# timosachsenberg/specpride

Measured on AMD Instinct MI355X. Metric: clusters/sec (whole node) for medoid + binned consensus, higher is better.
Workload: dtype f64; 1 GPU; configs[4]: full pipeline (bin-mean consensus + medoid representative) on a PRIDE-scale clustered dataset of ~10M spectra, U{2..50} spectra/cluster, ~200 peaks/spectrum; clusters=385000, clusters_this_rank=385000, spectra_this_rank=10008913, parallelism=cluster-sharded x1, launcher=single process, gather=none (1 GPU: results stay in HBM)

## Files before the change

### specpride_amd/csrc/bin_mean.hip

```cpp
#pragma once
#include <utility>

#include "spx_device.hpp"

namespace spx {

struct BinMeanParams {
  double minimum, maximum, binsize, inv_binsize;
  int32_t apply_quorum;
  int32_t n_words;
};

template <class PrefixT, class CountT = uint32_t>
struct BinMeanState {
  unsigned long long* bitmap;
  PrefixT* wprefix;
  CountT* cnt;
  float* acc_i;
  float* acc_m;
  uint32_t* owner;
  int32_t* soff;
  double* prec;
  int* votes;
  int32_t* xch;
// ... 432 lines not shown
    w[4 * k] = q.x; w[4 * k + 1] = q.y; w[4 * k + 2] = q.z; w[4 * k + 3] = q.w;
  }
  static_assert(BR_MDW32 == 4 * BM_BLOCK, "one b128 of medoid words per thread");
  const uint4 mq = reinterpret_cast<const uint4*>(L.u.b.mdbits)[threadIdx.x];
  const uint32_t mw[4] = {mq.x, mq.y, mq.z, mq.w};
  int local = 0, mlocal = 0;
#pragma unroll
  for (int k = 0; k < BR_WPT; ++k) local += __popc(w[k]);
#pragma unroll
  for (int k = 0; k < 4; ++k) mlocal += __popc(mw[k]);
  int total;
  const int packed = block_exclusive_scan<BM_BLOCK, int, true, false>(local | (mlocal << 16), L.tmp, total);
  int base = packed & 0xFFFF, mbase = (int)((uint32_t)packed >> 16);
  uint2* dst = reinterpret_cast<uint2*>(L.u.b.pre) + threadIdx.x * (BR_WPT / 4);
#pragma unroll
  for (int k = 0; k < BR_WPT / 4; ++k) {
    uint32_t p[4];
#pragma unroll
    for (int i = 0; i < 4; ++i) { p[i] = (uint32_t)base; base += __popc(w[4 * k + i]); }
    dst[k] = make_uint2(p[0] | (p[1] << 16), p[2] | (p[3] << 16));
  }
  uint32_t mp[4];
#pragma unroll
  for (int i = 0; i < 4; ++i) { mp[i] = (uint32_t)mbase; mbase += __popc(mw[i]); }
  reinterpret_cast<uint2*>(L.u.b.mdpre)[threadIdx.x] = make_uint2(mp[0] | (mp[1] << 16), mp[2] | (mp[3] << 16));
  lds_barrier();
  *md_total = (int)((uint32_t)total >> 16);
  return total & 0xFFFF;
}

struct MdSide {
  double tol, inv_tol;
  int out, K;
  int32_t rlo, rhi;
};

template <class F>
__device__ __forceinline__ void reg_steps(int n, F&& f) {
  unrolled_while(n, f, std::make_integer_sequence<int, BR_NMAX>{});
}

template <bool kMd>
__device__ __forceinline__ int32_t bin_mean_reg_path_t(const CsrView& v, const BinMeanParams& P, BinRegSmem& L,
                                                       int64_t c, const PeaksOut& out, double* prec_out,
                                                       int32_t* charge_out, int32_t (&code)[BR_NMAX], MdSide* md) {
  const int tid = threadIdx.x, lane = lane_id(), wid = wave_id();
  constexpr int KM = kMd ? SPX_BR_KM_MD : BR_KM;
  constexpr int PFA = kMd ? SPX_BR_PFA_MD : BR_PFA;
  const int64_t s0 = v.cluster_off[c], s1 = v.cluster_off[c + 1], n64 = s1 - s0;
  if (n64 < 1 || n64 > BR_NMAX || P.n_words > BM_WMAX) return kNotHere;
  const int n = (int)n64;
  const int64_t p0 = v.spec_off[s0], p1 = v.spec_off[s1];
  if (p1 == p0 || p1 - p0 >= (int64_t(1) << 28)) return kNotHere;
  const int jl = lane < n ? lane : n - 1;
  const int32_t rlo = (int32_t)(v.spec_off[s0 + jl] - p0), rhi = (int32_t)(v.spec_off[s0 + jl + 1] - p0);
  const int32_t z0 = v.charge[s0];
  const bool mine = lane < n;
  const int32_t zl = v.charge[s0 + jl];
  const double pl = v.prec_mz[s0 + jl];
  if (__ballot(mine & ((rhi - rlo) > BM_FASTLEN)) != 0ull) return kNotHere;
  if (__ballot(mine & (zl != z0)) != 0ull) {
    if (tid == 0) { out.count[c] = 0; prec_out[c] = __longlong_as_double(0x7ff8000000000000ll); charge_out[c] = 0; }
    return kMixedCharge;
  }
  if (wid == 0 && mine) L.prec[lane] = pl;
  if constexpr (kMd) {
    md->rlo = rlo;
    md->rhi = rhi;
    reinterpret_cast<uint4*>(L.u.b.mdbits)[tid] = make_uint4(0u, 0u, 0u, 0u);
  }
  {
    uint4* z = reinterpret_cast<uint4*>(L.u.b.bits) + tid * (BR_WPT / 4);
#pragma unroll
    for (int k = 0; k < BR_WPT / 4; ++k) z[k] = make_uint4(0u, 0u, 0u, 0u);
    if (tid < kWave) {
      L.u.b.bits[BR_W32 + tid] = 0u;
      L.u.b.pre[BR_W32 + tid] = (uint16_t)(BM_DCAP + tid);
    }
  }
  lds_barrier();
  SPX_STAMP2(1, -1);

  const int fpos = wid * (kWave - 1) + lane;
  const bool owner = lane < kWave - 1;
  const __amdgpu_buffer_rsrc_t rmz = bf_rsrc(v.mz + p0, (int)(p1 - p0));
  const __amdgpu_buffer_rsrc_t rit = bf_rsrc(v.inten + p0, (int)(p1 - p0));
  auto boffb = [&](int j) -> int {
    const int jj = j < n ? j : n - 1;
    return (__builtin_amdgcn_readlane(rlo, jj) + fpos) * 8;
  };

  double mk[KM > 0 ? KM : 1];
  uint32_t* bm32 = L.u.b.bits;
  int bad = 0, mdout = 0;
  {
    double ra[PFA];
    int rl[PFA];
    auto fetch = [&](int j, double& m, int& len) __attribute__((always_inline)) {
      const int jj = j < n ? j : n - 1;
      const int a = __builtin_amdgcn_readlane(rlo, jj), e = __builtin_amdgcn_readlane(rhi, jj);
      const int k = a + fpos;
      len = e - a;
      m = bf_load(rmz, k * 8, 0);
// ... 107 lines not shown
  lds_barrier();
  for (int d = tid; d < D; d += BM_BLOCK) L.u.acc[d] = BinAcc{0.0f, 0.0f, 0u, 0u};
  lds_barrier();
  SPX_STAMP2(3, 2);

  reg_steps(n, [&](auto jc) __attribute__((always_inline)) {
    constexpr int j = decltype(jc)::value;
    double m;
    const double it = ri[j % BR_PFC];
    if constexpr (j < KM) m = mk[j];
    else m = rm[j % BR_PFC];
    const int bo = boffb(j + BR_PFC);
    if constexpr (j + BR_PFC >= KM) rm[j % BR_PFC] = bf_load(rmz, bo, 0);
    ri[j % BR_PFC] = bf_load(rit, bo, 0);
    const int slot = kMd ? code[j] & 0xFFFF : code[j];
    if constexpr (kMd && (j & 1)) {
      code[j - 1] = (int32_t)(((uint32_t)code[j - 1] >> 16) | ((uint32_t)code[j] & 0xFFFF0000u));
    }
    BinAcc a = L.u.acc[slot];
    a.i = (float)((double)a.i + it);
    a.m = (float)((double)a.m + m);
    a.n += 1u;
    L.u.acc[slot] = a;
    lds_barrier();
  });
  SPX_STAMP2(4, 3);

  const uint32_t quorum = P.apply_quorum ? (uint32_t)((double)n * 0.25) + 1u : 1u;
  const int total = emit_striped_f([&](int d) { return L.u.acc[d].n; }, [&](int d) { return L.u.acc[d].i; },
                                   [&](int d) { return L.u.acc[d].m; }, L.wcnt, D, quorum, out.mz + p0,
                                   out.inten + p0);
  if (tid == 0) {
    out.count[c] = total;
    charge_out[c] = z0;
    prec_out[c] = pw_sum_small([&](int64_t j) { return L.prec[j]; }, n) / (double)n;
  }
  return kOk;
}

using BinHeadSmem = BinRegSmem;
__device__ __forceinline__ int32_t bin_mean_head_path(const CsrView& v, const BinMeanParams& P, BinHeadSmem& L,
                                                      int64_t c, const PeaksOut& out, double* prec_out,
                                                      int32_t* charge_out) {
  int32_t code[BR_NMAX];
  return bin_mean_reg_path_t<false>(v, P, L, c, out, prec_out, charge_out, code, nullptr);
}

__global__ __launch_bounds__(BM_BLOCK, SPX_BR_MINW) void bin_mean_reg_kernel(CsrView v, BinMeanParams P, PeaksOut out,
                                                                             double* prec_out, int32_t* charge_out,
                                                                             int32_t* status, StripedList rest) {
  __shared__ BinHeadSmem L;
  const int64_t c = blockIdx.x;
  SPX_STAMP(0);
  const int32_t st = bin_mean_head_path(v, P, L, c, out, prec_out, charge_out);
  SPX_STAMP(6);
  if (threadIdx.x == 0) {
    if (st != kNotHere) status[c] = st;
    if (st == kNotHere || st == kDeferred) striped_push(rest, (int32_t)c);
  }
}

__global__ __launch_bounds__(BM_BLOCK, SPX_BM_MINW) void bin_mean_lds_kernel(CsrView v, BinMeanParams P, PeaksOut out,
                                                                double* prec_out, int32_t* charge_out,
                                                                int32_t* status, const int32_t* list,
                                                                const int32_t* n_list, int32_t* deferred,
                                                                int32_t* n_deferred) {
  __shared__ BinMeanSmem L;
// ... 78 lines not shown
```

### specpride_amd/csrc/fused.hip

```cpp
#include "bin_mean.hip"
#include "medoid.hip"

namespace spx {

#ifndef SPX_FU_MINW
#define SPX_FU_MINW 5
#endif

union FusedSmem {
  BinHeadSmem b;
  MedoidRegSmem<MD_BLOCK, MR_UMAX, MD_KWMAX> m;
};
static_assert(BM_BLOCK == MD_BLOCK, "one workgroup shape for both bodies");

template <class Defer>
__device__ __forceinline__ void medoid_from_codes(const CsrView& v, int64_t* rep, double* totals_out,
                                                  MedoidRegSmem<MD_BLOCK, MR_UMAX, MD_KWMAX>& L, int64_t c,
                                                  const int32_t (&code)[BR_NMAX], const MdSide& md,
                                                  const Defer& defer) {
  const int tid = threadIdx.x, lane = lane_id(), wid = wave_id();
  const int64_t s0 = v.cluster_off[c];
  const int n = (int)(v.cluster_off[c + 1] - s0);
  if (n <= 1) {
    if (tid == 0) {
      rep[c] = n == 1 ? s0 : -1;
      if (totals_out && n == 1) totals_out[s0] = 0.0;
    }
    return;
  }
  const int KW = ((md.K + 63) / 64) | 1;
  if (KW > MD_KWMAX) {
    if (tid == 0) defer(c, s0, n);
    return;
  }
  if (tid <= n) L.soff[tid] = tid < n ? md.rlo : md.rhi;
  for (int w = tid; w < n * KW; w += MD_BLOCK) L.u.a.rows[w] = 0ull;
  __syncthreads();
  const uint32_t swz_nw = 2u * (uint32_t)KW;
  const uint32_t swz_m = swz_nw >= 32u ? 31u : (1u << (31 - __clz((int)swz_nw))) - 1u;
  const int fpos = wid * (kWave - 1) + lane;
  const bool owner = lane < kWave - 1;
  reg_steps(n, [&](auto jc) __attribute__((always_inline)) {
    constexpr int j = decltype(jc)::value;
    const int len = __builtin_amdgcn_readlane(md.rhi, j) - __builtin_amdgcn_readlane(md.rlo, j);
    if (owner & (fpos < len)) {
      uint32_t col;
      if constexpr (j & 1) col = (uint32_t)code[j - 1] >> 16;
      else col = j + 1 < n ? (uint32_t)code[j] & 0xFFFFu : (uint32_t)code[j] >> 16;
      uint32_t wq = (col >> 5) + (col & swz_m);
      wq = min(wq, wq - swz_nw);
      atomicOr(reinterpret_cast<uint32_t*>(&L.u.a.rows[__mul24(j, KW)]) + wq, 1u << (col & 31));
    }
  });
  SPX_STAMP2(-1, 5);
  medoid_tail<MD_BLOCK, MR_UMAX, MD_KWMAX>(L, n, KW, s0, c, rep, totals_out);
}

__global__ __launch_bounds__(BM_BLOCK, SPX_FU_MINW) void bin_mean_medoid_kernel(
    CsrView v, BinMeanParams PB, PeaksOut out, double* prec_out, int32_t* charge_out, int32_t* status,
    StripedList bm_rest, MedoidParams PM, int64_t* rep, double* totals_out, StripedList md_wide) {
  __shared__ FusedSmem L;
  const int64_t c = blockIdx.x;
  SPX_STAMP2(-1, 0);
  int32_t code[BR_NMAX];
  MdSide md{PM.tol, PM.inv_tol, 1, 0, 0, 0};
  const int32_t st = bin_mean_reg_path_t<true>(v, PB, L.b, c, out, prec_out, charge_out, code, &md);
  if (threadIdx.x == 0) {
    if (st != kNotHere) status[c] = st;
    if (st == kNotHere || st == kDeferred) striped_push(bm_rest, (int32_t)c);
  }
  SPX_STAMP2(-1, 4);
  __syncthreads();
  auto defer = [&](int64_t cc, int64_t, int) {
    rep[cc] = -4;
    striped_push(md_wide, (int32_t)cc);
  };
  if (st == kOk && !md.out) {
    medoid_from_codes(v, rep, totals_out, L.m, c, code, md, defer);
  } else {
    medoid_small_body<MD_BLOCK, MR_UMAX, MD_KWMAX>(v, PM, rep, totals_out, L.m, c, defer);
  }
}

__global__ __launch_bounds__(kWave) void handoff_count_kernel(const int32_t* bm_counts, const int32_t* md_counts,
                                                              int32_t* out) {
  const int l = threadIdx.x;
  const int32_t a = wave_sum(bm_counts[l * kListLine]);
  const int32_t b = wave_sum(md_counts[l * kListLine]);
  if (l == 0) {
    out[0] = a;
    out[1] = b;
  }
}

}
```

### specpride_amd/csrc/medoid.hip

```cpp
#pragma once
#include <type_traits>

#include "spx_device.hpp"

namespace spx {

struct MedoidParams {
  double tol, inv_tol;
};

constexpr int MD_BLOCK = 256;
constexpr int MD_NMAX = 64;
#ifndef SPX_MD_KWMAX
#define SPX_MD_KWMAX 27
#endif
#ifndef SPX_MD_MINW
#define SPX_MD_MINW 7
#endif
#ifndef SPX_MD_MFMA_NMIN
#define SPX_MD_MFMA_NMIN 32
#endif
constexpr int MD_KWMAX = SPX_MD_KWMAX;


// ... 101 lines not shown
constexpr int MR_UMAX = 48;
constexpr int MR_PMAX = MR_UMAX * MD_BLOCK;
constexpr int MR_WMAX = 512;
constexpr int MR_TRI = MD_NMAX * (MD_NMAX + 1) / 2;

constexpr int MW_BLOCK = 512;
constexpr int MW_UMAX = 64;
constexpr int MW_PMAX = MW_UMAX * MW_BLOCK;
constexpr int MW_KWMAX = 95;

template <int BLOCK, int UMAX, int KWMAX>
struct MedoidRegSmem {
  union {
    struct {
      unsigned long long bits[MR_WMAX];
      uint32_t pre[MR_WMAX];
      unsigned long long rows[MD_NMAX * KWMAX];
      unsigned long long sbits[UMAX * BLOCK / 64];
      uint8_t spre[UMAX * BLOCK / 64];
    } a;
    double d[MR_TRI];
    struct {
      double d[MR_TRI];
      double col[MD_NMAX];
    } t;
  } u;
  int32_t soff[MD_NMAX + 1];
  double totals[MD_NMAX];
  int tmp[BLOCK / kWave + 1];
  long long red[4];
  int votes[2 * (BLOCK / kWave)];
};

template <int BLOCK, int UMAX, int KWMAX>
__device__ __forceinline__ void medoid_tail(MedoidRegSmem<BLOCK, UMAX, KWMAX>& L, int n, int KW, int64_t s0,
                                            int64_t c, int64_t* rep, double* totals_out) {
  constexpr int PMAX = UMAX * BLOCK;
  const int tid = threadIdx.x, lane = lane_id(), wid = wave_id();
  static_assert(PMAX <= 65536, "md_dist_r's exact range");
  if (tid < n) {
    const int p = L.soff[tid + 1] - L.soff[tid];
    L.totals[tid] = p > 0 ? 1.0 / (double)p : 0.0;
  }
  __syncthreads();
  SPX_STAMP2(4, -1);

  auto row_start = [&](int i) { return i * n - (i * (i - 1)) / 2; };
  bool mfma_p4 = false;
  if constexpr (BLOCK == MD_BLOCK) mfma_p4 = n > SPX_MD_MFMA_NMIN;
  if (mfma_p4) {
  {
    const int fr = lane & 31, fh = lane >> 5;
    const int ntile = n > 32 ? 3 : 1;
    const bool work = wid < ntile;
    const int ta = wid == 2 ? 1 : 0, tb = wid == 0 ? 0 : 1;
    md_f32x16 acc;
#pragma unroll
    for (int q = 0; q < 16; ++q) acc[q] = 0.0f;
    if (work) {
      const int ra = ta * 32 + fr, rb = tb * 32 + fr;
      const unsigned long long* pa = L.u.a.rows + (ra < n ? ra : 0) * KW;
      const unsigned long long* pb = L.u.a.rows + (rb < n ? rb : 0) * KW;
      const unsigned long long ma = ra < n ? ~0ull : 0ull, mb = rb < n ? ~0ull : 0ull;
      unsigned long long wa = pa[0] & ma, wb = pb[0] & mb;
      for (int w = 0; w < KW; ++w) {
        const int wn = w + 1 < KW ? w + 1 : w;
        const unsigned long long na = pa[wn] & ma, nb = pb[wn] & mb;
        acc = __builtin_amdgcn_mfma_scale_f32_32x32x64_f8f6f4(md_frag4(wa, fh), md_frag4(wb, fh), acc, 4, 4, 0, 0,
                                                              0, 0);
        wa = na;
        wb = nb;
      }
    }
    __syncthreads();
    if (work) {
      const int j = tb * 32 + fr;
#pragma unroll
      for (int q = 0; q < 16; ++q) {
// ... 10 lines not shown
    constexpr int PPT = (MD_NMAX * (MD_NMAX + 1) / 2 + BLOCK - 1) / BLOCK;
    const int NP = n * (n + 1) / 2;
    uint32_t pc[PPT];
    int pij[PPT];
#pragma unroll
    for (int q = 0; q < PPT; ++q) {
      const int p = tid + q * BLOCK;
      pc[q] = 0u;
      pij[q] = -1;
      if (p < NP) {
        const float b2 = 2.0f * n + 1.0f;
        int i = (int)((b2 - sqrtf(b2 * b2 - 8.0f * (float)p)) * 0.5f);
        i = i < 0 ? 0 : (i > n - 1 ? n - 1 : i);
        while (i > 0 && row_start(i) > p) --i;
        while (i + 1 < n && row_start(i + 1) <= p) ++i;
        const int j = i + (p - row_start(i));
        uint32_t cnt = 0;
        for (int w = 0; w < KW; ++w) cnt += (uint32_t)__popcll(L.u.a.rows[i * KW + w] & L.u.a.rows[j * KW + w]);
        pc[q] = cnt;
        pij[q] = i << 8 | j;
      }
    }
    __syncthreads();
#pragma unroll
    for (int q = 0; q < PPT; ++q) {
      if (pij[q] >= 0) {
        const int i = pij[q] >> 8, j = pij[q] & 0xff;
        L.u.d[row_start(i) + j - i] =
            md_dist_r(pc[q], L.soff[i + 1] - L.soff[i], L.totals[i], L.soff[j + 1] - L.soff[j], L.totals[j]);
      }
    }
  }
  __syncthreads();

  SPX_STAMP2(5, 6);
  const bool colside = wid == 1;
  const int i5 = lane;
  const bool valid5 = i5 < n;
  double sum = 0.0;
  if (tid < 2 * kWave) {
    const int i = i5;
    const bool valid = valid5;
    const int lim = n >= 8 ? n - n % 8 : 0;
    auto term = [&](int j) -> double {
      const bool use = valid && (colside ? j <= i : j >= i);
      return use ? (colside ? L.u.d[row_start(j) + i - j] : L.u.d[row_start(i) + j - i]) : 0.0;
    };
    double r[8];
#pragma unroll
    for (int k = 0; k < 8; ++k) r[k] = 0.0;
    for (int j0 = 0; j0 < lim; j0 += 8) {
      double v[8];
#pragma unroll
      for (int k = 0; k < 8; ++k) v[k] = term(j0 + k);
#pragma unroll
      for (int k = 0; k < 8; ++k) r[k] += v[k];
    }
    sum = ((r[0] + r[1]) + (r[2] + r[3])) + ((r[4] + r[5]) + (r[6] + r[7]));
    for (int j = lim; j < n; ++j) sum += term(j);
    sum = 0.0 + sum;
    if (colside && valid) L.u.t.col[i] = sum;
  }
  lds_barrier();
  if (wid == 0 && valid5) {
    const double t = (sum + L.u.t.col[i5]) / (double)n;
    L.totals[i5] = t;
// ... 1205 lines not shown
```

### specpride_amd/csrc/spx_api.hip

```cpp
#include <hip/hip_runtime.h>

#include <algorithm>
#include <atomic>
#include <cmath>
#include <cstdio>
#include <cstdlib>
#include <cstring>
#include <functional>
#include <mutex>
#include <utility>
#include <vector>

#include "../../include/specpride.h"

#if defined(SPX_DG_NOMZ) || defined(SPX_DG_NOBAR) || defined(SPX_DG_P3LANE) || defined(SPX_DG_NOMIRROR) || \
    defined(SPX_GR_DIAG) || defined(SPX_QF_DIAG) || defined(SPX_BR_FOLD) || defined(SPX_BF_RING) ||       \
    defined(SPX_BF_REVERSE)
#error "diagnostic / rejected variants are not part of libspecpride_hip (see git history)"
#endif
#if defined(SPX_GA_FLAT4) || defined(SPX_GA_FLAT6) || defined(SPX_GA_HASH) || defined(SPX_GA_HASH2) ||     \
    defined(SPX_GA_HASH3) || defined(SPX_GA_NOFILT) || defined(SPX_GA_TPERM) || defined(SPX_GA_GBATCH) ||  \
    defined(SPX_GA_HYBRID) || defined(SPX_GA_P3INT) || defined(SPX_GA_BSKIP) || defined(SPX_GA_P2B) ||     \
    defined(SPX_GA_EARLY) || defined(SPX_GA_DEFERBIG) || defined(SPX_MD_MFMA) || defined(SPX_MD_P5L) ||    \
    defined(SPX_MD_RECIP) || defined(SPX_MD_R32) || defined(SPX_MD_MBC) || defined(SPX_MD_L1RUNS) ||       \
// ... 298 lines not shown
  W.scl = w.take<spx::SplitCluster>(C);
  W.range_cap = split_range_cap(csr);
  W.ranges = w.take<spx::SplitRange>((size_t)W.range_cap);
  W.meta = w.take<spx::SegMeta>(C);
  W.seg_in = w.take<int32_t>(C);
  const int64_t q_bound = std::min<int64_t>(csr->n_clusters, csr->n_spectra / 129 + csr->n_peaks / 4097 + 2);
  const int32_t task_cap = (int32_t)std::min<int64_t>(csr->n_spectra + 1, INT32_MAX);
  const int32_t tile_cap = (int32_t)std::min<int64_t>(q_bound * (spx::BM_WMAX / spx::Q_TILEW) + 1, INT32_MAX);
  const int32_t unit_cap = (int32_t)std::min<int64_t>(csr->n_peaks / 32 + q_bound + 1, INT32_MAX);
  carve_kept_fold(w, W.fold, C, task_cap, tile_cap, unit_cap);
  W.n_task_cap = csr->n_spectra / spx::SG_SB + csr->n_clusters + 1;
  W.task_cl = w.take<int32_t>((size_t)W.n_task_cap);
  W.n_tile_cap = csr->n_peaks / spx::SG_TILE + csr->n_clusters + 1;
  W.tile_cl = w.take<int32_t>((size_t)W.n_tile_cap);
  W.arena_bytes = seg_arena_bytes(csr, params);
  W.arena = w.take<char>((size_t)W.arena_bytes);
  const bool in = bin_mean_intake_possible(info);
  W.fold_in.list = w.take<int32_t>(in ? C : 1);
  carve_kept_fold(w, W.fold_in, in ? C : 1, in ? task_cap : 1, in ? tile_cap : 1, in ? unit_cap : 2);
  W.scratch = w.base + w.used;
  W.fold.n_list = W.counters + kBmcDeferred;
  W.fold.n_tasks = W.counters + kBmcFoldTasks;
  W.fold.n_tiles = W.counters + kBmcFoldTiles;
  W.fold.n_units = W.counters + kBmcFoldUnits;
  W.fold_in.n_list = W.counters + kBmcInDeferred;
  W.fold_in.n_tasks = W.counters + kBmcInTasks;
  W.fold_in.n_tiles = W.counters + kBmcInTiles;
  W.fold_in.n_units = W.counters + kBmcInUnits;
  return W;
}

struct BinMeanHead {
  int (*launch)(void* ctx, const spx::CsrView& V, const spx::BinMeanParams& P, const spx::PeaksOut& O,
                double* prec_out, int32_t* charge_out, int32_t* status, const spx::StripedList& rest, hipStream_t s);
  void* ctx;
};

int bin_mean_validate(const spx_csr* csr, const spx_bin_params* params, const spx_batch_info* info,
                      const spx_peaks_out* out, const double* prec_out, const int32_t* charge_out,
                      const int32_t* status, const void* workspace, size_t workspace_bytes) {
  if (!csr_ok(csr) || !params || !info || !out || !out->count || !prec_out || !charge_out || !status)
    return fail(SPX_EINVAL, "spx_bin_mean: null argument");
  if (!(params->binsize > 0) || !(params->maximum > params->minimum))
    return fail(SPX_EINVAL, "spx_bin_mean: need binsize > 0 and maximum > minimum");
  if (csr->n_peaks && (!out->mz || !out->inten)) return fail(SPX_EINVAL, "spx_bin_mean: null output arrays");
  const size_t need = spx_bin_mean_workspace_size(csr, params, info);
  if (!workspace || workspace_bytes < need) return fail(SPX_ENOSPACE, "spx_bin_mean: workspace too small");
  return SPX_SUCCESS;
}

enum BmStage { kBmAll = 0, kBmFront = 1, kBmChain = 2, kBmHead = 3, kBmTail = 4 };

enum FoldPart { kFoldAll, kFoldSetup, kFoldRest };

int bin_mean_impl(const spx_csr* csr, const spx_bin_params* params, const spx_batch_info* info,
                  spx_peaks_out* out, double* prec_out, int32_t* charge_out, int32_t* status, void* workspace,
                  size_t workspace_bytes, void* stream, int stage, const BinMeanHead* head) {
  if (stage < kBmAll || stage > kBmTail) return fail(SPX_EINVAL, "bin_mean_impl: stage must be 0..4 (BmStage)");
  if (int rc = bin_mean_validate(csr, params, info, out, prec_out, charge_out, status, workspace, workspace_bytes))
    return rc;
  const int64_t C = csr->n_clusters;
  if (C == 0) return SPX_SUCCESS;
  hipStream_t s = reinterpret_cast<hipStream_t>(stream);
  Carver w{static_cast<char*>(workspace), 0};
  const BinMeanWs W = carve_bin_mean(w, csr, params, info);
  auto cnt = [&](BmCounter slot) { return W.counters + slot; };

// ... 22 lines not shown
    int rc = SPX_LAUNCH(bin_mean_q_tally_kernel, gqt, bsg, q, V, P, K.meta, W.arena, K.task_cl, K.n_tasks, K.task_cap);
    if (!rc) rc = SPX_LAUNCH(bin_mean_q_count_kernel, dim3((unsigned)std::max(1, std::min(K.tile_cap, 8192))), bsg, q,
                             K.meta, W.arena, K.tile_cl, K.n_tiles, K.tile_cap);
    if (!rc) rc = SPX_LAUNCH(bin_mean_q_plan_kernel, gcl, bsg, q, K.n_list, K.meta, W.arena, W.bump, W.arena_bytes,
                             K.unit_cl, K.n_units, K.unit_cap);
    if (!rc) rc = SPX_LAUNCH(bin_mean_q_place_kernel, gqt, bsg, q, V, P, K.meta, W.arena, K.task_cl, K.n_tasks,
                             K.task_cap);
    if (!rc) rc = SPX_LAUNCH(bin_mean_q_fold_kernel, dim3((unsigned)std::max(1, std::min(K.unit_cap, 2048))),
                             dim3(spx::QF_BLOCK), q, K.meta, W.arena, K.unit_cl, K.n_units, K.unit_cap);
    if (!rc) rc = SPX_LAUNCH(bin_mean_q_emit_kernel, gcl, bsg, q, V, O, prec_out, charge_out, status, K.n_list, K.meta,
                             W.arena, W.seg_in, cnt(kBmcSegIn), W.glist, cnt(kBmcGlobal));
    return rc;
  };
  const bool intake = stage == kBmAll && !head && P.apply_quorum && kept_fold_enabled() &&
                      bin_mean_intake_possible(info);
  SideFork side("spx_bin_mean");
  auto global_pass = [&]() {
    return SPX_LAUNCH(bin_mean_global_kernel, dim3((unsigned)bin_mean_fallback_grid(C, params, dcap)), bbm, s, V, P, O,
                      prec_out, charge_out, status, W.glist, cnt(kBmcGlobal), W.scratch,
                      spx::bin_mean_slice_bytes(P.n_words, dcap), (int)std::min<int64_t>(dcap, INT32_MAX));
  };
  if (stage == kBmAll || stage == kBmFront || stage == kBmHead) {
    if (hipMemsetAsync(W.counters, 0, W.zeroed, s) != hipSuccess) return check_launch("spx_bin_mean memset");
    if (intake) {
      if (int rc = side.begin(s)) return rc;
      if (int rc = SPX_LAUNCH(bin_mean_intake_kernel, dim3((unsigned)std::min<int64_t>((C + 255) / 256, 1024)),
                              dim3(256), side.stream(), V, P, W.fold_in.list, W.fold_in.n_list))
        return rc;
      if (int rc = kept_fold(W.fold_in, side.stream(), kFoldSetup)) return rc;
      if (int rc = side.mark_mid()) return rc;
      if (int rc = side.wait_mid(s)) return rc;
    }
    if (head) {
      if (int rc = head->launch(head->ctx, V, P, O, prec_out, charge_out, status, W.rest, s)) return rc;
    } else {
      if (int rc = SPX_LAUNCH_TIMED(ProfScope(kProfBinMeanReg, s), bin_mean_reg_kernel, dim3((unsigned)C), bbm, s, V, P,
                                    O, prec_out, charge_out, status, W.rest))
        return rc;
    }
    if (intake) {
      if (int rc = kept_fold(W.fold_in, side.stream(), kFoldRest)) return rc;
      if (int rc = side.mark_join()) return rc;
    }
  }
  if (stage == kBmHead) return SPX_SUCCESS;
  if (stage != kBmChain) {
    if (int rc = SPX_LAUNCH(bin_mean_wide_kernel, gcl, dim3(spx::BW_BLOCK), s, V, P, O, prec_out, charge_out, status,
                            W.rest, W.fold.list, W.fold.n_list, W.glist, cnt(kBmcGlobal), intake ? 1 : 0))
      return rc;
  }
  if (stage == kBmFront) return global_pass();
  if (stage == kBmChain) {
    if (hipMemsetAsync(cnt(kBmcGlobal), 0, sizeof(int32_t), s) != hipSuccess)
      return check_launch("spx_bin_mean memset");
  }
  if (int rc = kept_fold(W.fold, s, kFoldAll)) return rc;
  if (intake)
    if (int rc = side.wait_join(s)) return rc;
  const dim3 gtask((unsigned)std::max<int64_t>(1, std::min<int64_t>(W.n_task_cap, 8192)));
  const dim3 gtile((unsigned)std::max<int64_t>(1, std::min<int64_t>(W.n_tile_cap, 8192)));
  int rc = SPX_LAUNCH(bin_mean_seg_setup_kernel, gcl, bsg, s, V, P, O, prec_out, charge_out, status, W.seg_in,
                      cnt(kBmcSegIn), W.meta, W.arena, W.bump, W.arena_bytes, W.task_cl, cnt(kBmcSegTasks));
  if (!rc) rc = SPX_LAUNCH(bin_mean_seg_occupy_kernel, gtask, bsg, s, V, P, W.meta, W.arena, W.task_cl,
                           cnt(kBmcSegTasks));
  if (!rc) rc = SPX_LAUNCH(bin_mean_seg_prefix_kernel, gcl, bsg, s, V, P, O, prec_out, charge_out, status,
                           cnt(kBmcSegIn), W.meta, W.arena, W.bump, W.arena_bytes, W.tile_cl, cnt(kBmcSegTiles));
  if (!rc) rc = SPX_LAUNCH(bin_mean_seg_mask_kernel, gtask, bsg, s, V, P, W.meta, W.arena, W.task_cl,
// ... 224 lines not shown
  const bool intake = part == kMdAll && params->large_path;
  SideFork side("spx_medoid");
  if (intake)
    if (int rc = side.begin(s)) return rc;
  if (part == kMdAll) {
    if (int rc = SPX_LAUNCH_TIMED(ProfScope(kProfMedoidReg, s), medoid_reg_kernel, dim3((unsigned)C), blk, s, V, P, rep,
                                  totals, W.wide, intake ? 1 : 0))
      return rc;
  }
  if (intake) {
    if (int rc = SPX_LAUNCH(medoid_intake_kernel, dim3((unsigned)std::min<int64_t>((C + 255) / 256, 1024)), dim3(256),
                            side.stream(), V, rep, W.in.def, W.in.n_def, W.in.meta))
      return rc;
    if (int rc = large_path(W.in, side.stream())) return rc;
    if (int rc = side.mark_join()) return rc;
  }
  if (int rc = SPX_LAUNCH(medoid_wide_kernel, dim3((unsigned)std::max<int64_t>(1, std::min<int64_t>(C, 1024))),
                          dim3(spx::MW_BLOCK), s, V, P, rep, totals, W.wide, W.late.def, W.late.n_def, W.late.meta))
    return rc;
  if (!params->large_path) return SPX_SUCCESS;
  if (int rc = large_path(W.late, s)) return rc;
  if (intake) return side.wait_join(s);
  return SPX_SUCCESS;
}

struct FusedCtx {
  const MedoidHead* md;
  int64_t* rep;
  double* totals;
  int64_t C;
  const int32_t* bm_counts;
};

int fused_head(void* ctx, const spx::CsrView& V, const spx::BinMeanParams& P, const spx::PeaksOut& O, double* prec_out,
               int32_t* charge_out, int32_t* status, const spx::StripedList& rest, hipStream_t s) {
  FusedCtx& F = *static_cast<FusedCtx*>(ctx);
  F.bm_counts = rest.counts;
  return SPX_LAUNCH_TIMED(ProfScope(kProfBinMeanMedoid, s), bin_mean_medoid_kernel, dim3((unsigned)F.C),
                          dim3(spx::BM_BLOCK), s, V, P, O, prec_out, charge_out, status, rest, F.md->P, F.rep, F.totals,
                          F.md->wide);
}

struct CosineWs {
  int32_t *n_def, *def;
  char* scratch;
};

CosineWs carve_cosine(Carver& w, int64_t n_clusters) {
  CosineWs W;
  W.n_def = w.take<int32_t>(1);
  W.def = w.take<int32_t>((size_t)std::max<int64_t>(n_clusters, 1));
  W.scratch = w.base + w.used;
  return W;
}

}

extern "C" {

int spx_abi_version(void) { return SPX_ABI_VERSION; }

#ifdef SPX_STAMPS
int spx_debug_stamps(void* dev_ptr) {
  return hipMemcpyToSymbol(HIP_SYMBOL(spx::g_spx_stamps), &dev_ptr, sizeof(dev_ptr)) == hipSuccess ? 0 : SPX_EHIP;
}
#endif
const char* spx_last_error(void) { return g_err; }

int spx_profile_enable(int on) {
  std::lock_guard<std::mutex> lock(g_prof_mu);
  for (auto& p : g_prof) {
    for (auto& ab : p.pending) {
      (void)hipEventSynchronize(ab.second);
// ... 429 lines not shown
```

### specpride_amd/csrc/spx_device.hpp

```cpp
#pragma once
#include <utility>

#include <hip/hip_runtime.h>

#include <type_traits>
#include <stdint.h>

#ifdef SPX_DEBUG
#include <stdio.h>
#define SPX_GUARD(cond, ...)        \
  if (!(cond)) {                    \
    printf(__VA_ARGS__);            \
  } else
#else
#define SPX_GUARD(cond, ...)
#endif

namespace spx {

constexpr int kWave = 64;

#ifdef SPX_STAMPS
__device__ unsigned long long* g_spx_stamps;
#define SPX_STAMP(k)                                                                           \
  do {                                                                                         \
    if (threadIdx.x == 0 && g_spx_stamps)                                                      \
      g_spx_stamps[(size_t)blockIdx.x * 8 + (k)] = (unsigned long long)__builtin_amdgcn_s_memtime(); \
  } while (0)
#else
#define SPX_STAMP(k) \
  do {               \
  } while (0)
#endif
#ifdef SPX_STAMPS_FU
#define SPX_STAMP2(other, fu) \
  do {                        \
    if ((fu) >= 0) SPX_STAMP((fu) < 0 ? 0 : (fu)); \
  } while (0)
#else
#define SPX_STAMP2(other, fu) \
  do {                        \
    if ((other) >= 0) SPX_STAMP((other) < 0 ? 0 : (other)); \
  } while (0)
#endif

struct CsrView {
  int64_t n_clusters, n_spectra, n_peaks;
  const int64_t* __restrict__ cluster_off;
  const int64_t* __restrict__ spec_off;
  const double* __restrict__ mz;
  const double* __restrict__ inten;
  const double* __restrict__ prec_mz;
  const int32_t* __restrict__ charge;
  const double* __restrict__ rt;
};

struct PeaksOut {
  double* __restrict__ mz;
  double* __restrict__ inten;
  int64_t* __restrict__ count;
};

enum : int32_t { kOk = 0, kMixedCharge = 1, kNoGap = 2, kEmpty = 3, kNonFinite = 4, kDeferred = 100 };

__device__ __forceinline__ double bf_load(__amdgpu_buffer_rsrc_t r, int voff, int soff) {
  return __builtin_bit_cast(double, __builtin_amdgcn_raw_buffer_load_b64(r, voff, soff, 0));
}
// ... 407 lines not shown
```

Baseline: 34.61 million clusters/s.

## Make fused bin-mean/medoid kernel persistent with prefetched cluster headers

The fused bin-mean+medoid kernel now launches an occupancy-sized persistent grid. Blocks pull clusters from an atomic work queue and double-buffer a per-cluster header (offsets, charges, precursor m/z) in LDS. The last wave prefetches the next cluster's CSR metadata during the medoid tail through hooks, hiding global-load latency at cluster start and removing per-block launch overhead. The risks are atomic contention on the queue head, extra LDS use that may lower occupancy, and more complex control flow using goto and asm barriers.

```diff
diff --git a/specpride_amd/csrc/bin_mean.hip b/specpride_amd/csrc/bin_mean.hip
--- a/specpride_amd/csrc/bin_mean.hip
+++ b/specpride_amd/csrc/bin_mean.hip
@@ -488,8 +488,22 @@
 struct MdSide {
   double tol, inv_tol;
   int out, K;
-  int32_t rlo, rhi;
 };
+
+struct RegHeader {
+  int64_t s0, p0, p1;
+  int32_t c;
+  int32_t n;
+  int32_t rel[BR_NMAX + 2];
+  int32_t charge[BR_NMAX];
+  double prec[BR_NMAX];
+};
+
+__device__ __forceinline__ int64_t uniform64(int64_t x) {
+  const uint64_t lo = (uint32_t)__builtin_amdgcn_readfirstlane((int)(uint32_t)(uint64_t)x);
+  const uint64_t hi = (uint32_t)__builtin_amdgcn_readfirstlane((int)(uint32_t)((uint64_t)x >> 32));
+  return (int64_t)(lo | (hi << 32));
+}
 
 template <class F>
 __device__ __forceinline__ void reg_steps(int n, F&& f) {
@@ -499,32 +513,31 @@
 template <bool kMd>
 __device__ __forceinline__ int32_t bin_mean_reg_path_t(const CsrView& v, const BinMeanParams& P, BinRegSmem& L,
                                                        int64_t c, const PeaksOut& out, double* prec_out,
-                                                       int32_t* charge_out, int32_t (&code)[BR_NMAX], MdSide* md) {
+                                                       int32_t* charge_out, int32_t (&code)[BR_NMAX], MdSide* md,
+                                                       const RegHeader* hd = nullptr) {
   const int tid = threadIdx.x, lane = lane_id(), wid = wave_id();
   constexpr int KM = kMd ? SPX_BR_KM_MD : BR_KM;
   constexpr int PFA = kMd ? SPX_BR_PFA_MD : BR_PFA;
-  const int64_t s0 = v.cluster_off[c], s1 = v.cluster_off[c + 1], n64 = s1 - s0;
+  const int hn = kMd ? __builtin_amdgcn_readfirstlane(hd->n) : 0;
+  const int64_t s0 = kMd ? int64_t(0) : v.cluster_off[c], s1 = kMd ? (int64_t)hn : v.cluster_off[c + 1], n64 = s1 - s0;
   if (n64 < 1 || n64 > BR_NMAX || P.n_words > BM_WMAX) return kNotHere;
   const int n = (int)n64;
-  const int64_t p0 = v.spec_off[s0], p1 = v.spec_off[s1];
+  const int64_t p0 = kMd ? uniform64(hd->p0) : v.spec_off[s0], p1 = kMd ? uniform64(hd->p1) : v.spec_off[s1];
   if (p1 == p0 || p1 - p0 >= (int64_t(1) << 28)) return kNotHere;
   const int jl = lane < n ? lane : n - 1;
-  const int32_t rlo = (int32_t)(v.spec_off[s0 + jl] - p0), rhi = (int32_t)(v.spec_off[s0 + jl + 1] - p0);
-  const int32_t z0 = v.charge[s0];
+  const int32_t rlo = kMd ? hd->rel[jl] : (int32_t)(v.spec_off[s0 + jl] - p0),
+                rhi = kMd ? hd->rel[jl + 1] : (int32_t)(v.spec_off[s0 + jl + 1] - p0);
+  const int32_t z0 = kMd ? hd->charge[0] : v.charge[s0];
   const bool mine = lane < n;
-  const int32_t zl = v.charge[s0 + jl];
-  const double pl = v.prec_mz[s0 + jl];
+  const int32_t zl = kMd ? hd->charge[jl] : v.charge[s0 + jl];
+  const double pl = kMd ? hd->prec[jl] : v.prec_mz[s0 + jl];
   if (__ballot(mine & ((rhi - rlo) > BM_FASTLEN)) != 0ull) return kNotHere;
   if (__ballot(mine & (zl != z0)) != 0ull) {
     if (tid == 0) { out.count[c] = 0; prec_out[c] = __longlong_as_double(0x7ff8000000000000ll); charge_out[c] = 0; }
     return kMixedCharge;
   }
   if (wid == 0 && mine) L.prec[lane] = pl;
-  if constexpr (kMd) {
-    md->rlo = rlo;
-    md->rhi = rhi;
-    reinterpret_cast<uint4*>(L.u.b.mdbits)[tid] = make_uint4(0u, 0u, 0u, 0u);
-  }
+  if constexpr (kMd) reinterpret_cast<uint4*>(L.u.b.mdbits)[tid] = make_uint4(0u, 0u, 0u, 0u);
   {
     uint4* z = reinterpret_cast<uint4*>(L.u.b.bits) + tid * (BR_WPT / 4);
 #pragma unroll
@@ -698,7 +711,7 @@
                                    out.inten + p0);
   if (tid == 0) {
     out.count[c] = total;
-    charge_out[c] = z0;
+    charge_out[c] = kMd ? hd->charge[0] : z0;
     prec_out[c] = pw_sum_small([&](int64_t j) { return L.prec[j]; }, n) / (double)n;
   }
   return kOk;
diff --git a/specpride_amd/csrc/fused.hip b/specpride_amd/csrc/fused.hip
--- a/specpride_amd/csrc/fused.hip
+++ b/specpride_amd/csrc/fused.hip
@@ -5,6 +5,9 @@
 
 #ifndef SPX_FU_MINW
 #define SPX_FU_MINW 5
+#endif
+#ifndef SPX_FU_STATIC
+#define SPX_FU_STATIC 0
 #endif
 
 union FusedSmem {
@@ -13,36 +16,103 @@
 };
 static_assert(BM_BLOCK == MD_BLOCK, "one workgroup shape for both bodies");
 
+struct FusedPrefetch {
+  uint32_t tc;
+  int64_t toff, tso;
+  int32_t tz;
+  double tp;
+
+  __device__ __forceinline__ void claim(uint32_t* head, uint32_t& k) {
+    tc = 0u;
+#if SPX_FU_STATIC
+    tc = blockIdx.x + k * gridDim.x;
+#else
+    if (lane_id() == 0) tc = atomicAdd(head, 1u);
+#endif
+    ++k;
+  }
+  __device__ __forceinline__ void offsets(const CsrView& v, RegHeader* H) {
+    const uint32_t c = (uint32_t)__builtin_amdgcn_readfirstlane((int)tc);
+    const int32_t cn = (int64_t)c < v.n_clusters ? (int32_t)c : -1;
+    if (lane_id() == 0) H->c = cn;
+    toff = 0;
+    if (cn >= 0) toff = v.cluster_off[(int64_t)cn + (lane_id() != 0)];
+  }
+  __device__ __forceinline__ void spectra(const CsrView& v, RegHeader* H) {
+    if (__builtin_amdgcn_readfirstlane(H->c) < 0) return;
+    const int64_t s0 = readlane64(toff, 0);
+    const int64_t n64 = readlane64(toff, 1) - s0;
+    const int32_t n = n64 >= 1 && n64 <= BR_NMAX ? (int32_t)n64 : BR_NMAX + 1;
+    if (lane_id() == 0) {
+      H->s0 = s0;
+      H->n = n;
+    }
+    if (n > BR_NMAX) return;
+    const int j = lane_id() < n ? lane_id() : n, jj = lane_id() < n ? lane_id() : n - 1;
+    tso = v.spec_off[s0 + j];
+    tz = v.charge[s0 + jj];
+    tp = v.prec_mz[s0 + jj];
+  }
+  __device__ __forceinline__ void commit(RegHeader* H) {
+    if (__builtin_amdgcn_readfirstlane(H->c) < 0) return;
+    const int n = __builtin_amdgcn_readfirstlane(H->n);
+    if (n > BR_NMAX) return;
+    const int lane = lane_id();
+    const int64_t p0 = readlane64(tso, 0);
+    if (lane == 0) H->p0 = p0;
+    if (lane == n) H->p1 = tso;
+    if (lane <= n) H->rel[lane] = (int32_t)(tso - p0);
+    if (lane < n) {
+      H->charge[lane] = tz;
+      H->prec[lane] = tp;
+    }
+  }
+  __device__ __forceinline__ void all(const CsrView& v, uint32_t* head, uint32_t& k, RegHeader* H) {
+    claim(head, k);
+    offsets(v, H);
+    spectra(v, H);
+    commit(H);
+  }
+};
+
+__device__ __forceinline__ bool fused_prefetch_wave() {
+  return __builtin_amdgcn_readfirstlane(wave_id()) == BM_BLOCK / kWave - 1;
+}
+
 template <class Defer>
-__device__ __forceinline__ void medoid_from_codes(const CsrView& v, int64_t* rep, double* totals_out,
+__device__ __forceinline__ bool medoid_from_codes(int64_t* rep, double* totals_out,
                                                   MedoidRegSmem<MD_BLOCK, MR_UMAX, MD_KWMAX>& L, int64_t c,
                                                   const int32_t (&code)[BR_NMAX], const MdSide& md,
-                                                  const Defer& defer) {
+                                                  const Defer& defer, const RegHeader& hd, FusedPrefetch& pf,
+                                                  const CsrView& v, uint32_t* head, uint32_t& k, RegHeader* Hn) {
   const int tid = threadIdx.x, lane = lane_id(), wid = wave_id();
-  const int64_t s0 = v.cluster_off[c];
-  const int n = (int)(v.cluster_off[c + 1] - s0);
+  const int64_t s0 = hd.s0;
+  const int n = __builtin_amdgcn_readfirstlane(hd.n);
   if (n <= 1) {
     if (tid == 0) {
       rep[c] = n == 1 ? s0 : -1;
       if (totals_out && n == 1) totals_out[s0] = 0.0;
     }
-    return;
+    return false;
   }
   const int KW = ((md.K + 63) / 64) | 1;
   if (KW > MD_KWMAX) {
     if (tid == 0) defer(c, s0, n);
-    return;
-  }
-  if (tid <= n) L.soff[tid] = tid < n ? md.rlo : md.rhi;
+    return false;
+  }
+  const int jl = lane < n ? lane : n - 1;
+  const int32_t rlo = hd.rel[jl], rhi = hd.rel[jl + 1];
+  if (tid <= n) L.soff[tid] = tid < n ? rlo : rhi;
   for (int w = tid; w < n * KW; w += MD_BLOCK) L.u.a.rows[w] = 0ull;
   __syncthreads();
+  if (fused_prefetch_wave()) pf.claim(head, k);
   const uint32_t swz_nw = 2u * (uint32_t)KW;
   const uint32_t swz_m = swz_nw >= 32u ? 31u : (1u << (31 - __clz((int)swz_nw))) - 1u;
   const int fpos = wid * (kWave - 1) + lane;
   const bool owner = lane < kWave - 1;
   reg_steps(n, [&](auto jc) __attribute__((always_inline)) {
     constexpr int j = decltype(jc)::value;
-    const int len = __builtin_amdgcn_readlane(md.rhi, j) - __builtin_amdgcn_readlane(md.rlo, j);
+    const int len = __builtin_amdgcn_readlane(rhi, j) - __builtin_amdgcn_readlane(rlo, j);
     if (owner & (fpos < len)) {
       uint32_t col;
       if constexpr (j & 1) col = (uint32_t)code[j - 1] >> 16;
@@ -53,33 +123,83 @@
     }
   });
   SPX_STAMP2(-1, 5);
-  medoid_tail<MD_BLOCK, MR_UMAX, MD_KWMAX>(L, n, KW, s0, c, rep, totals_out);
-}
-
-__global__ __launch_bounds__(BM_BLOCK, SPX_FU_MINW) void bin_mean_medoid_kernel(
-    CsrView v, BinMeanParams PB, PeaksOut out, double* prec_out, int32_t* charge_out, int32_t* status,
-    StripedList bm_rest, MedoidParams PM, int64_t* rep, double* totals_out, StripedList md_wide) {
+  medoid_tail<MD_BLOCK, MR_UMAX, MD_KWMAX>(L, n, KW, s0, c, rep, totals_out,
+                                           [&](int at) __attribute__((always_inline)) {
+                                             if (!fused_prefetch_wave()) return;
+                                             if (at == 0) pf.offsets(v, Hn);
+                                             else pf.spectra(v, Hn);
+                                           });
+  if (fused_prefetch_wave()) pf.commit(Hn);
+  return true;
+}
+
+struct FusedArgs {
+  CsrView v;
+  BinMeanParams PB;
+  PeaksOut out;
+  double* prec_out;
+  int32_t* charge_out;
+  int32_t* status;
+  StripedList bm_rest;
+  MedoidParams PM;
+  int64_t* rep;
+  double* totals_out;
+  StripedList md_wide;
+  uint32_t* queue;
+};
+
+__global__ __launch_bounds__(BM_BLOCK, SPX_FU_MINW) void bin_mean_medoid_kernel(FusedArgs) {
   __shared__ FusedSmem L;
-  const int64_t c = blockIdx.x;
+  __shared__ RegHeader H[2];
+  using ArgsPtr = const FusedArgs __attribute__((address_space(4)))*;
+  ArgsPtr ap = (ArgsPtr)__builtin_amdgcn_kernarg_segment_ptr();
+  uint32_t k = 0u;
+  if (fused_prefetch_wave()) {
+    FusedPrefetch pf{};
+    pf.all(((const FusedArgs*)ap)->v, ((const FusedArgs*)ap)->queue, k, &H[0]);
+  }
+  int cur = 0;
+  int never = 0;
+  asm volatile("" : "+s"(never));
+  if (never) {
+    asm volatile("" : "+s"(never));
+    goto next_cluster;
+  }
+cluster : {
+  asm volatile("" : "+s"(ap));
+  const FusedArgs& A = *(const FusedArgs*)ap;
+  const RegHeader& hd = H[cur];
+  RegHeader* Hn = &H[cur ^ 1];
+  lds_barrier();
+  const int32_t c32 = __builtin_amdgcn_readfirstlane(hd.c);
+  if (c32 < 0) return;
+  const int64_t c = c32;
   SPX_STAMP2(-1, 0);
+  auto defer = [&](int64_t cc, int64_t, int) {
+    A.rep[cc] = -4;
+    striped_push(A.md_wide, (int32_t)cc);
+  };
   int32_t code[BR_NMAX];
-  MdSide md{PM.tol, PM.inv_tol, 1, 0, 0, 0};
-  const int32_t st = bin_mean_reg_path_t<true>(v, PB, L.b, c, out, prec_out, charge_out, code, &md);
+  MdSide md{A.PM.tol, A.PM.inv_tol, 1, 0};
+  const int32_t st = bin_mean_reg_path_t<true>(A.v, A.PB, L.b, c, A.out, A.prec_out, A.charge_out, code, &md, &hd);
   if (threadIdx.x == 0) {
-    if (st != kNotHere) status[c] = st;
-    if (st == kNotHere || st == kDeferred) striped_push(bm_rest, (int32_t)c);
+    if (st != kNotHere) A.status[c] = st;
+    if (st == kNotHere || st == kDeferred) striped_push(A.bm_rest, (int32_t)c);
   }
   SPX_STAMP2(-1, 4);
   __syncthreads();
-  auto defer = [&](int64_t cc, int64_t, int) {
-    rep[cc] = -4;
-    striped_push(md_wide, (int32_t)cc);
-  };
+  FusedPrefetch pf{};
+  bool fetched = false;
   if (st == kOk && !md.out) {
-    medoid_from_codes(v, rep, totals_out, L.m, c, code, md, defer);
+    fetched = medoid_from_codes(A.rep, A.totals_out, L.m, c, code, md, defer, hd, pf, A.v, A.queue, k, Hn);
   } else {
-    medoid_small_body<MD_BLOCK, MR_UMAX, MD_KWMAX>(v, PM, rep, totals_out, L.m, c, defer);
-  }
+    medoid_small_body<MD_BLOCK, MR_UMAX, MD_KWMAX>(A.v, A.PM, A.rep, A.totals_out, L.m, c, defer);
+  }
+  if (!fetched && fused_prefetch_wave()) pf.all(A.v, A.queue, k, Hn);
+}
+next_cluster:
+  cur ^= 1;
+  goto cluster;
 }
 
 __global__ __launch_bounds__(kWave) void handoff_count_kernel(const int32_t* bm_counts, const int32_t* md_counts,
diff --git a/specpride_amd/csrc/medoid.hip b/specpride_amd/csrc/medoid.hip
--- a/specpride_amd/csrc/medoid.hip
+++ b/specpride_amd/csrc/medoid.hip
@@ -157,9 +157,13 @@
   int votes[2 * (BLOCK / kWave)];
 };
 
-template <int BLOCK, int UMAX, int KWMAX>
+struct MedoidNoHook {
+  __device__ __forceinline__ void operator()(int) const {}
+};
+template <int BLOCK, int UMAX, int KWMAX, class Hook = MedoidNoHook>
 __device__ __forceinline__ void medoid_tail(MedoidRegSmem<BLOCK, UMAX, KWMAX>& L, int n, int KW, int64_t s0,
-                                            int64_t c, int64_t* rep, double* totals_out) {
+                                            int64_t c, int64_t* rep, double* totals_out,
+                                            const Hook& hook = Hook{}) {
   constexpr int PMAX = UMAX * BLOCK;
   const int tid = threadIdx.x, lane = lane_id(), wid = wave_id();
   static_assert(PMAX <= 65536, "md_dist_r's exact range");
@@ -169,6 +173,7 @@
   }
   __syncthreads();
   SPX_STAMP2(4, -1);
+  if constexpr (!std::is_same<Hook, MedoidNoHook>::value) hook(0);
 
   auto row_start = [&](int i) { return i * n - (i * (i - 1)) / 2; };
   bool mfma_p4 = false;
@@ -245,6 +250,7 @@
     }
   }
   __syncthreads();
+  if constexpr (!std::is_same<Hook, MedoidNoHook>::value) hook(1);
 
   SPX_STAMP2(5, 6);
   const bool colside = wid == 1;
diff --git a/specpride_amd/csrc/spx_api.hip b/specpride_amd/csrc/spx_api.hip
--- a/specpride_amd/csrc/spx_api.hip
+++ b/specpride_amd/csrc/spx_api.hip
@@ -354,7 +354,8 @@
 
 struct BinMeanHead {
   int (*launch)(void* ctx, const spx::CsrView& V, const spx::BinMeanParams& P, const spx::PeaksOut& O,
-                double* prec_out, int32_t* charge_out, int32_t* status, const spx::StripedList& rest, hipStream_t s);
+                double* prec_out, int32_t* charge_out, int32_t* status, const spx::StripedList& rest, int32_t* queue,
+                hipStream_t s);
   void* ctx;
 };
 
@@ -443,7 +444,8 @@
       if (int rc = side.wait_mid(s)) return rc;
     }
     if (head) {
-      if (int rc = head->launch(head->ctx, V, P, O, prec_out, charge_out, status, W.rest, s)) return rc;
+      if (int rc = head->launch(head->ctx, V, P, O, prec_out, charge_out, status, W.rest, cnt(kBmcUnused), s))
+        return rc;
     } else {
       if (int rc = SPX_LAUNCH_TIMED(ProfScope(kProfBinMeanReg, s), bin_mean_reg_kernel, dim3((unsigned)C), bbm, s, V, P,
                                     O, prec_out, charge_out, status, W.rest))
@@ -734,13 +736,47 @@
   const int32_t* bm_counts;
 };
 
+int64_t fused_grid(int64_t C) {
+  static std::mutex mu;
+  static int64_t slots[64];
+  int dev = 0;
+  if (hipGetDevice(&dev) != hipSuccess || dev < 0) return -1;
+  int64_t g = 0;
+  {
+    std::lock_guard<std::mutex> lock(mu);
+    int64_t& cached = slots[dev < 64 ? dev : 63];
+    if (dev >= 64 || cached == 0) {
+      int cus = 0, per_cu = 0;
+      if (hipDeviceGetAttribute(&cus, hipDeviceAttributeMultiprocessorCount, dev) != hipSuccess ||
+          hipOccupancyMaxActiveBlocksPerMultiprocessor(&per_cu, spx::bin_mean_medoid_kernel, spx::BM_BLOCK, 0) !=
+              hipSuccess ||
+          cus < 1 || per_cu < 1)
+        return -1;
+      cached = (int64_t)cus * per_cu;
+    }
+    g = cached;
+  }
+  if (const char* e = std::getenv("SPX_FU_GRID")) {
+    const long long v = std::strtoll(e, nullptr, 10);
+    if (v > 0) g = std::min<int64_t>(g, v);
+  }
+  return std::max<int64_t>(1, std::min(g, C));
+}
+
 int fused_head(void* ctx, const spx::CsrView& V, const spx::BinMeanParams& P, const spx::PeaksOut& O, double* prec_out,
-               int32_t* charge_out, int32_t* status, const spx::StripedList& rest, hipStream_t s) {
+               int32_t* charge_out, int32_t* status, const spx::StripedList& rest, int32_t* queue, hipStream_t s) {
   FusedCtx& F = *static_cast<FusedCtx*>(ctx);
   F.bm_counts = rest.counts;
-  return SPX_LAUNCH_TIMED(ProfScope(kProfBinMeanMedoid, s), bin_mean_medoid_kernel, dim3((unsigned)F.C),
-                          dim3(spx::BM_BLOCK), s, V, P, O, prec_out, charge_out, status, rest, F.md->P, F.rep, F.totals,
-                          F.md->wide);
+  const int64_t grid = fused_grid(F.C);
+  if (grid < 1) {
+    if (int rc = check_launch("spx_bin_mean_medoid occupancy query")) return rc;
+    return fail(SPX_EHIP, "spx_bin_mean_medoid: occupancy query failed");
+  }
+  if (F.C > (int64_t)INT32_MAX - grid) return fail(SPX_EINVAL, "spx_bin_mean_medoid: too many clusters");
+  const spx::FusedArgs A{V,        P,     O,        prec_out,   charge_out, status, rest, F.md->P,
+                         F.rep,    F.totals, F.md->wide, reinterpret_cast<uint32_t*>(queue)};
+  return SPX_LAUNCH_TIMED(ProfScope(kProfBinMeanMedoid, s), bin_mean_medoid_kernel, dim3((unsigned)grid),
+                          dim3(spx::BM_BLOCK), s, A);
 }
 
 struct CosineWs {
diff --git a/specpride_amd/csrc/spx_device.hpp b/specpride_amd/csrc/spx_device.hpp
--- a/specpride_amd/csrc/spx_device.hpp
+++ b/specpride_amd/csrc/spx_device.hpp
@@ -32,7 +32,23 @@
   do {               \
   } while (0)
 #endif
-#ifdef SPX_STAMPS_FU
+#if defined(SPX_STAMPS) && defined(SPX_STAMPS_FU)
+#define SPX_STAMP_AT(row, k)                                                                    \
+  do {                                                                                          \
+    if (threadIdx.x == 0 && g_spx_stamps)                                                       \
+      g_spx_stamps[(size_t)(row) * 8 + (k)] = (unsigned long long)__builtin_amdgcn_s_memtime(); \
+  } while (0)
+#ifdef SPX_STAMPS_FU_SETUP
+#define SPX_STAMP_FU_SLOT(other, fu) ((other) == 1 && (fu) < 0 ? 1 : ((fu) == 1 ? -1 : (fu)))
+#else
+#define SPX_STAMP_FU_SLOT(other, fu) (fu)
+#endif
+#define SPX_STAMP2(other, fu)                                                          \
+  do {                                                                                 \
+    if (SPX_STAMP_FU_SLOT(other, fu) >= 0)                                             \
+      SPX_STAMP_AT(c, SPX_STAMP_FU_SLOT(other, fu) < 0 ? 0 : SPX_STAMP_FU_SLOT(other, fu)); \
+  } while (0)
+#elif defined(SPX_STAMPS_FU)
 #define SPX_STAMP2(other, fu) \
   do {                        \
     if ((fu) >= 0) SPX_STAMP((fu) < 0 ? 0 : (fu)); \
```

Measured after the change: 37.22 million clusters/s, median of 6. +7.5%, better.
